# shizukutanaka/Otedama

Measured on AMD Instinct MI355X. Metric: hashes/sec (whole node) SHA-256d + scrypt at 1/2/4/8 MI355X; p50 share latency, higher is better.
Workload: dtype u32

## Files before the change

### csrc/bindings.cpp

```cpp
#include <pybind11/pybind11.h>
#include <pybind11/stl.h>

#include <array>
#include <atomic>
#include <cstring>
#include <stdexcept>
#include <thread>
#include <tuple>

#include "otedama/aead.h"
#include "otedama/job.h"
#include "otedama/runtime.h"
#include "otedama/trace.h"
#include "otedama/sha256.h"
#include "otedama/sv2_frame.h"
#include "otedama/clock_bounds.h"
#include "otedama/launch_plan.h"
#include "otedama/search_launch.h"
#include "otedama/share_job.h"
#include "otedama/work_queue.h"
#include "otedama/x11.h"

namespace py = pybind11;
using namespace otedama;

namespace {

std::string need(const py::bytes& b, size_t n, const char* what) {
  std::string s = b;
  if (s.size() != n) throw std::invalid_argument(std::string(what) + ": expected " + std::to_string(n) + " bytes");
  return s;
}

py::bytes to_bytes(const uint8_t* p, size_t n) { return py::bytes(reinterpret_cast<const char*>(p), n); }

std::shared_ptr<JobTemplate> make_job(const py::dict& d) {
  auto j = std::make_shared<JobTemplate>();
  auto get = [&](const char* k) -> py::object {
    if (d.contains(k)) return py::object(d[k]);
    return py::none();
  };
  std::string hdr = need(d["header"].cast<py::bytes>(), 80, "header");
  std::memcpy(j->header, hdr.data(), 80);
  std::string tgt = need(d["target"].cast<py::bytes>(), 32, "target");
  std::memcpy(j->target, tgt.data(), 32);
  if (!get("epoch").is_none()) j->epoch = d["epoch"].cast<uint64_t>();
  if (!get("job_id").is_none()) j->job_id = d["job_id"].cast<std::string>();
  if (!get("channel_id").is_none()) j->channel_id = d["channel_id"].cast<uint32_t>();
  if (!get("algo").is_none()) {
    auto a = d["algo"].cast<std::string>();
    if (a == "sha256d") j->algo = Algo::kSha256d;
    else if (a == "scrypt") j->algo = Algo::kScrypt;
    else if (a == "x11") j->algo = Algo::kX11;
    else throw std::invalid_argument("unsupported algo for the native miner: " + a);
  }
  if (!get("version_mask").is_none()) j->version_mask = d["version_mask"].cast<uint32_t>();
  if (!get("ntime_roll").is_none()) j->ntime_roll = d["ntime_roll"].cast<uint32_t>();
  if (!get("coinb1").is_none()) {
    j->has_coinbase = true;
    std::string c1 = d["coinb1"].cast<py::bytes>(), c2 = d["coinb2"].cast<py::bytes>();
    std::string e1 = d["extranonce1"].cast<py::bytes>();
    j->coinb1.assign(c1.begin(), c1.end());
    j->coinb2.assign(c2.begin(), c2.end());
    j->extranonce1.assign(e1.begin(), e1.end());
    j->extranonce2_size = d["extranonce2_size"].cast<uint32_t>();
    for (auto& br : d["merkle_branches"].cast<py::list>()) {
      std::string b = br.cast<py::bytes>();
      j->merkle_branches.emplace_back(b.begin(), b.end());
    }
  }
  if (!get("variant_start").is_none()) j->variant_start = d["variant_start"].cast<uint64_t>();
  if (!get("variant_stride").is_none()) j->variant_stride = d["variant_stride"].cast<uint64_t>();
  if (j->variant_stride == 0) j->variant_stride = 1;
  return j;
}

py::list shares_to_list(std::vector<ShareRecord>&& v) {
  py::list out;
  for (auto& s : v) {
    py::dict d;
    d["epoch"] = s.epoch;
    d["job_id"] = s.job_id;
    d["channel_id"] = s.channel_id;
    d["nonce"] = s.nonce;
    d["ntime"] = s.ntime;
    d["version"] = s.version;
    d["extranonce2"] = s.extranonce2;
    d["extranonce2_size"] = s.extranonce2_size;
    d["hash"] = to_bytes(s.hash, 32);
    d["device_id"] = s.device_id;
    d["found_at"] = s.found_at;
    d["device_found_at"] = s.device_found_at;
    out.append(d);
  }
  return out;
}

py::dict stats_to_dict(const MinerStats& s) {
  py::dict d;
  d["hashes"] = s.hashes;
  d["candidates"] = s.candidates;
  d["shares"] = s.shares;
  d["dropped"] = s.dropped;
  d["launches"] = s.launches;
  d["rejected_candidates"] = s.rejected_candidates;
  d["variant_launches"] = s.variant_launches;
  d["busy_seconds"] = s.busy_seconds;
  d["faulted"] = s.faulted;
  d["error"] = s.error;
  d["variant_next"] = s.variant_next;
  d["variant_epoch"] = s.variant_epoch;
  d["job_switches"] = s.job_switches;
  d["last_job_switch_ms"] = s.last_job_switch_ms;
  d["job_switch_ms"] = s.job_switch_ms;
  d["work_started"] = s.work_started;
  d["reserved_cus"] = s.reserved_cus;
  d["ring_overflow"] = s.ring_overflow;
  d["verify_dropped"] = s.verify_dropped;
  d["verify_queue_peak"] = s.verify_queue_peak;
  d["launch_hashes"] = s.launch_hashes;
  d["aborted_launches"] = s.aborted_launches;
  d["ring_hits"] = s.ring_hits;
  d["clock_calib_rtt_us"] = s.clock_calib_rtt_us;
  d["clock_samples"] = s.clock_samples;
  d["host_abort"] = s.host_abort;
  d["hashes_done_at_s"] = s.hashes_done_at_s;
  {
    py::dict ph;
    for (const auto& kv : s.startup_ms) ph[py::str(kv.first)] = kv.second;
    d["startup_ms"] = ph;
    py::dict rs;
    for (const auto& kv : s.startup_rss_mb) rs[py::str(kv.first)] = kv.second;
    d["startup_rss_mb"] = rs;
  }
  return d;
}

}

PYBIND11_MODULE(_native, m) {
  m.doc() = "Otedama MI355X native runtime (gfx950 HIP kernels + C++ host runtime)";

  m.def("cpu_has_sha_ni", &cpu_has_sha_ni);
  m.def("sha256", [](const py::bytes& b) {
    std::string s = b; uint8_t o[32];
    sha256(reinterpret_cast<const uint8_t*>(s.data()), s.size(), o);
    return to_bytes(o, 32);
  });
  m.def("sha256d", [](const py::bytes& b) {
    std::string s = b; uint8_t o[32];
    { py::gil_scoped_release r; sha256d(reinterpret_cast<const uint8_t*>(s.data()), s.size(), o); }
    return to_bytes(o, 32);
  });
  m.def("hmac_sha256", [](const py::bytes& k, const py::bytes& msg) {
    std::string ks = k, ms = msg; uint8_t o[32];
    hmac_sha256(reinterpret_cast<const uint8_t*>(ks.data()), ks.size(),
                reinterpret_cast<const uint8_t*>(ms.data()), ms.size(), o);
    return to_bytes(o, 32);
  });
  m.def("aead_seal", [](int kind, const py::bytes& key, const py::bytes& nonce, const py::bytes& plain,
                        const py::bytes& aad) {
    std::string out = aead_seal(static_cast<AeadKind>(kind), key, nonce, plain, aad);
    return py::bytes(out);
  }, py::arg("kind"), py::arg("key"), py::arg("nonce"), py::arg("plain"), py::arg("aad") = py::bytes());
  m.def("aead_open", [](int kind, const py::bytes& key, const py::bytes& nonce, const py::bytes& sealed,
                        const py::bytes& aad) -> py::object {
    std::string out;
    if (!aead_open(static_cast<AeadKind>(kind), key, nonce, sealed, aad, &out)) return py::none();
    return py::bytes(out);
  }, py::arg("kind"), py::arg("key"), py::arg("nonce"), py::arg("sealed"), py::arg("aad") = py::bytes());
  m.attr("SCRYPT_COOP") = kScryptCoop;
  m.attr("SCRYPT_LANE_W8") = kScryptLaneW8;
  m.attr("SCRYPT_COOP2") = kScryptCoop2;
  m.attr("SCRYPT_COOP_SPLIT") = kScryptCoopSplit;
  m.attr("AEAD_AES256GCM") = 0;
  m.attr("AEAD_CHACHA20POLY1305") = 1;
  m.def("scrypt_1024_1_1_batch", [](const std::vector<py::bytes>& hs) {
    std::vector<std::string> in;
    for (const auto& h : hs) in.push_back(need(h, 80, "header"));
    std::vector<std::array<uint8_t, 32>> out(in.size());
    std::vector<const uint8_t*> ip;
    std::vector<uint8_t*> op;
    for (size_t i = 0; i < in.size(); ++i) {
      ip.push_back(reinterpret_cast<const uint8_t*>(in[i].data()));
      op.push_back(out[i].data());
    }
    {
      py::gil_scoped_release r;
      scrypt_1024_1_1_batch(int(in.size()), ip.data(), op.data());
    }
    py::list res;
    for (const auto& o : out) res.append(to_bytes(o.data(), 32));
    return res;
  });
  m.def("scrypt_1024_1_1", [](const py::bytes& h) {
    std::string s = need(h, 80, "header"); uint8_t o[32];
    { py::gil_scoped_release r; scrypt_1024_1_1(reinterpret_cast<const uint8_t*>(s.data()), o); }
    return to_bytes(o, 32);
  });
  m.def("_clock_bounds", [](double window, const std::vector<std::pair<double, double>>& samples) {
    ClockBounds cb(window);
    std::vector<double> out;
    for (const auto& s : samples) out.push_back(cb.add(s.first, s.second));
    return out;
  });
  m.def("_launch_plan_rules", [](uint64_t batch_nonces, uint32_t target_hi, bool capped, int sha_variants, int run,
                                 const std::string& reserve_cus, int ncu) {
    const ShaLayout lay = pick_layout(sha_variants, run);
    const CuMask cm = parse_reserved_cus(reserve_cus.c_str(), ncu);
    py::dict d;
    d["batch"] = normalize_batch(batch_nonces);
    d["cap"] = launch_cap_hashes(target_hi, capped);
    d["layout"] = py::make_tuple(lay.nvar, lay.use_v);
    d["cu_mask"] = cm.words;
    d["reserved"] = cm.reserved;
    return d;
  }, py::arg("batch_nonces") = 0, py::arg("target_hi") = 0, py::arg("capped") = true, py::arg("sha_variants") = 1,
     py::arg("run") = 1, py::arg("reserve_cus") = "", py::arg("ncu") = 256);
  m.def("_launch_plan_walk", [](const std::string& kind, uint64_t batch, uint64_t cap, int nvar, uint64_t lanes,
                                uint64_t start, size_t max_launches, uint64_t variant_start, uint64_t variant_stride) {
    const LaunchKind lk = kind == "scrypt" ? LaunchKind::kScrypt : kind == "x11" ? LaunchKind::kX11
                        : kind == "v" ? LaunchKind::kVersionParallel : kind == "k" ? LaunchKind::kVariantK
                        : kind == "single" ? LaunchKind::kSingle
                        : throw std::invalid_argument("kind: scrypt, x11, v, k or single");
    if (start >= kNonceSpace) throw std::invalid_argument("start must be below 2^32");
    SearchCursor c;
    c.nonce_off = start;
    std::vector<std::tuple<uint64_t, uint64_t, uint64_t>> launches;
    while (c.k == 0 && launches.size() < max_launches) {
      const uint64_t base = c.nonce_off, count = launch_count(lk, batch, cap, nvar, lanes, c.nonce_off);
      c.advance(count, nvar);
      launches.emplace_back(base, count, c.variant_next(variant_start, variant_stride, nvar));
    }
    return py::make_tuple(launches, c.k);
  }, py::arg("kind"), py::arg("batch"), py::arg("cap"), py::arg("nvar") = 1, py::arg("lanes") = 0,
     py::arg("start") = 0, py::arg("max_launches") = size_t(1) << 20, py::arg("variant_start") = 0,
     py::arg("variant_stride") = 1);
  m.def("_work_queue_flood", [](size_t cap, size_t n, bool hash_each, size_t batch) {
    BoundedWorkQueue<std::array<uint8_t, 80>> q(cap);
    std::atomic<uint64_t> processed{0};
    uint64_t accepted = 0;
    {
      py::gil_scoped_release r;
      std::thread consumer([&] {
        if (batch > 1) {
          std::vector<std::array<uint8_t, 80>> items;
          std::vector<const uint8_t*> ip;
          std::vector<std::array<uint8_t, 32>> outs(batch);
          std::vector<uint8_t*> op;
          for (auto& o : outs) op.push_back(o.data());
          while (items.clear(), q.pop_many(&items, batch) > 0) {
            ip.clear();
            for (const auto& it : items) ip.push_back(it.data());
            if (hash_each) scrypt_1024_1_1_batch(int(items.size()), ip.data(), op.data());
            processed.fetch_add(items.size());
          }
          return;
        }
        std::array<uint8_t, 80> h;
        uint8_t out[32];
        while (q.pop(&h)) {
          if (hash_each) scrypt_1024_1_1(h.data(), out);
          processed.fetch_add(1);
        }
      });
      for (size_t i = 0; i < n; ++i) {
        std::array<uint8_t, 80> h{};
        std::memcpy(h.data() + 76, &i, 4);
        if (q.push(std::move(h))) ++accepted;
      }
      q.stop(~size_t(0));
      consumer.join();
    }
    py::dict d;
    d["accepted"] = accepted;
    d["refused"] = q.refused();
    d["peak"] = q.peak();
    d["processed"] = processed.load();
    return d;
  }, py::arg("cap"), py::arg("n"), py::arg("hash_each") = true, py::arg("batch") = 1);
  m.attr("X11_STAGES") = kX11StageCount;
  m.def("x11", [](const py::bytes& msg) {
    std::string s = msg; uint8_t o[32];
    { py::gil_scoped_release r; x11::x11(reinterpret_cast<const uint8_t*>(s.data()), s.size(), o, nullptr); }
    return to_bytes(o, 32);
  }, py::arg("msg"));
  m.def("x11_trace", [](const py::bytes& msg) {
    std::string s = msg; uint8_t o[32], t[64 * kX11StageCount];
    x11::x11(reinterpret_cast<const uint8_t*>(s.data()), s.size(), o, t);
    return to_bytes(t, sizeof t);
  }, py::arg("msg"), "The 11 intermediate 64-byte digests of the X11 chain, concatenated.");
  m.def("x11_stage", [](int i, const py::bytes& msg) {
    if (i < 0 || i >= kX11StageCount) throw std::invalid_argument("stage must be in [0, 11)");
    std::string s = msg; uint8_t o[64];
    x11::stage(i, reinterpret_cast<const uint8_t*>(s.data()), s.size(), o);
    return to_bytes(o, 64);
  }, py::arg("stage"), py::arg("msg"));
  m.def("x11_luffa_sbox_selfcheck", &x11::luffa_sbox_selfcheck);
  m.def(
      "sv2_scan",
      [](py::buffer b, uint32_t max_frame) {
        py::buffer_info info = b.request();
        if (info.itemsize != 1 || info.ndim != 1) throw std::invalid_argument("sv2_scan: need a contiguous byte buffer");
        const size_t n = (size_t)info.size;
        if (n > 0xFFFFFFFFull) throw std::invalid_argument("sv2_scan: buffer larger than 4 GiB");
        std::vector<Sv2FrameRec> recs(n / kSv2HeaderSize + 1);
        size_t consumed = 0, k = 0;
        int status = kSv2Ok;
        {
          py::gil_scoped_release nogil;
          k = sv2_scan(static_cast<const uint8_t*>(info.ptr), n, max_frame, recs.data(), recs.size(), &consumed,
                       &status);
        }
        py::list frames(k);
        for (size_t i = 0; i < k; ++i) {
          const Sv2FrameRec& r = recs[i];
          frames[i] = py::make_tuple(r.extension_type, r.msg_type, r.offset, r.length);
        }
        return py::make_tuple(frames, consumed, status);
      },
      py::arg("buf"), py::arg("max_frame"),
      "Split complete SV2 frames: ([(extension_type, msg_type, payload_offset, payload_length)], consumed, status)");
  m.def("cpu_scan_sha256d", [](const py::bytes& h, const py::bytes& t, uint32_t start, uint64_t count) {
    std::string hs = need(h, 80, "header"), ts = need(t, 32, "target");
    std::vector<uint32_t> hits;
    {
      py::gil_scoped_release r;
      hits = cpu_scan_sha256d(reinterpret_cast<const uint8_t*>(hs.data()), reinterpret_cast<const uint8_t*>(ts.data()),
                              start, count);
    }
    return hits;
  }, py::arg("header"), py::arg("target"), py::arg("start"), py::arg("count"));
  m.def("cpu_scan_method", &cpu_scan_method);
  m.def("_cpu_scan_lanes", [](int lanes, const py::bytes& h, const py::bytes& t, uint32_t start, uint64_t count) {
    std::string hs = need(h, 80, "header"), ts = need(t, 32, "target");
    std::vector<uint32_t> hits;
    {
      py::gil_scoped_release r;
      hits = cpu_scan_sha256d_lanes(lanes, reinterpret_cast<const uint8_t*>(hs.data()),
                                    reinterpret_cast<const uint8_t*>(ts.data()), start, count);
    }
    return hits;
  });
  m.def("merkle_root", [](const py::dict& job, uint64_t en2) {
    auto j = make_job(job); uint8_t root[32];
    merkle_root_from_coinbase(*j, en2, root);
    return to_bytes(root, 32);
  });
  m.def("variant_header", [](const py::dict& job, uint64_t v) {
    auto j = make_job(job);
    uint8_t hdr[80]; uint32_t ver, nt; uint64_t en2;
    j->variant_header(v, hdr, &ver, &nt, &en2);
// ... 218 lines not shown
```

### csrc/kernels/cdna_bitops.h

```cpp
#pragma once
#include <hip/hip_runtime.h>

#include <cstdint>

namespace otedama_dev {

__device__ __forceinline__ uint32_t ror(uint32_t x, uint32_t n) { return __builtin_amdgcn_alignbit(x, x, n); }
__device__ __forceinline__ uint32_t rol(uint32_t x, uint32_t n) { return __builtin_amdgcn_alignbit(x, x, 32 - n); }

__device__ __forceinline__ uint32_t xor3(uint32_t a, uint32_t b, uint32_t c, bool lane_varying = true) {
  if (lane_varying) {
    uint32_t r;
    asm("v_bitop3_b32 %0, %1, %2, %3 bitop3:0x96" : "=v"(r) : "v"(a), "v"(b), "v"(c));
    return r;
  }
  return a ^ b ^ c;
}
__device__ __forceinline__ uint32_t ch(uint32_t e, uint32_t f, uint32_t g) {
  uint32_t r;
  asm("v_bitop3_b32 %0, %1, %2, %3 bitop3:0xca" : "=v"(r) : "v"(e), "v"(f), "v"(g));
  return r;
}
__device__ __forceinline__ uint32_t maj(uint32_t a, uint32_t b, uint32_t c) {
  uint32_t r;
  asm("v_bitop3_b32 %0, %1, %2, %3 bitop3:0xe8" : "=v"(r) : "v"(a), "v"(b), "v"(c));
  return r;
}

__device__ __forceinline__ uint32_t bS0(uint32_t a) { return xor3(ror(a, 2), ror(a, 13), ror(a, 22)); }
__device__ __forceinline__ uint32_t bS1(uint32_t e) { return xor3(ror(e, 6), ror(e, 11), ror(e, 25)); }
__device__ __forceinline__ uint32_t ss0(uint32_t x, bool v = true) { return xor3(ror(x, 7), ror(x, 18), x >> 3, v); }
__device__ __forceinline__ uint32_t ss1(uint32_t x, bool v = true) { return xor3(ror(x, 17), ror(x, 19), x >> 10, v); }

__device__ __forceinline__ constexpr uint32_t sha256_k(int i) {
  constexpr uint32_t k[64] = {
      0x428a2f98, 0x71374491, 0xb5c0fbcf, 0xe9b5dba5, 0x3956c25b, 0x59f111f1, 0x923f82a4, 0xab1c5ed5,
      0xd807aa98, 0x12835b01, 0x243185be, 0x550c7dc3, 0x72be5d74, 0x80deb1fe, 0x9bdc06a7, 0xc19bf174,
      0xe49b69c1, 0xefbe4786, 0x0fc19dc6, 0x240ca1cc, 0x2de92c6f, 0x4a7484aa, 0x5cb0a9dc, 0x76f988da,
      0x983e5152, 0xa831c66d, 0xb00327c8, 0xbf597fc7, 0xc6e00bf3, 0xd5a79147, 0x06ca6351, 0x14292967,
      0x27b70a85, 0x2e1b2138, 0x4d2c6dfc, 0x53380d13, 0x650a7354, 0x766a0abb, 0x81c2c92e, 0x92722c85,
      0xa2bfe8a1, 0xa81a664b, 0xc24b8b70, 0xc76c51a3, 0xd192e819, 0xd6990624, 0xf40e3585, 0x106aa070,
      0x19a4c116, 0x1e376c08, 0x2748774c, 0x34b0bcb5, 0x391c0cb3, 0x4ed8aa4a, 0x5b9cca4f, 0x682e6ff3,
      0x748f82ee, 0x78a5636f, 0x84c87814, 0x8cc70208, 0x90befffa, 0xa4506ceb, 0xbef9a3f7, 0xc67178f2};
  return k[i];
}

constexpr uint32_t kSha256IVd[8] = {0x6a09e667, 0xbb67ae85, 0x3c6ef372, 0xa54ff53a,
                                    0x510e527f, 0x9b05688c, 0x1f83d9ab, 0x5be0cd19};

__device__ __forceinline__ void sha256_compress(uint32_t st[8], const uint32_t msg[16]) {
  uint32_t W[64];
#pragma unroll
  for (int i = 0; i < 16; ++i) W[i] = msg[i];
  uint32_t a = st[0], b = st[1], c = st[2], d = st[3], e = st[4], f = st[5], g = st[6], h = st[7];
#pragma unroll
  for (int t = 0; t < 64; ++t) {
    if (t >= 16) W[t] = ss1(W[t - 2]) + W[t - 7] + ss0(W[t - 15]) + W[t - 16];
    const uint32_t t1 = h + bS1(e) + ch(e, f, g) + (sha256_k(t) + W[t]);
    const uint32_t t2 = bS0(a) + maj(a, b, c);
    h = g; g = f; f = e; e = d + t1; d = c; c = b; b = a; a = t1 + t2;
  }
  st[0] += a; st[1] += b; st[2] += c; st[3] += d; st[4] += e; st[5] += f; st[6] += g; st[7] += h;
}

}
```

### csrc/kernels/scrypt_search.hip

```cpp
#include <hip/hip_runtime.h>

#include <cstdint>

#include "cdna_bitops.h"
#include "hitsink_dev.h"
#include "scrypt_pbkdf_dev.h"
#include <cstdlib>
#include <cstring>

#include "otedama/job.h"
#include "otedama/search_launch.h"

namespace {

using namespace otedama_dev;
using namespace otedama_dev::scryptk;

__device__ __forceinline__ void salsa20_8(uint32_t B[16]) {
  uint32_t x0 = B[0], x1 = B[1], x2 = B[2], x3 = B[3], x4 = B[4], x5 = B[5], x6 = B[6], x7 = B[7];
  uint32_t x8 = B[8], x9 = B[9], x10 = B[10], x11 = B[11], x12 = B[12], x13 = B[13], x14 = B[14], x15 = B[15];
#pragma unroll
  for (int i = 0; i < 8; i += 2) {
    x4 ^= rol(x0 + x12, 7);   x8 ^= rol(x4 + x0, 9);    x12 ^= rol(x8 + x4, 13);   x0 ^= rol(x12 + x8, 18);
    x9 ^= rol(x5 + x1, 7);    x13 ^= rol(x9 + x5, 9);   x1 ^= rol(x13 + x9, 13);   x5 ^= rol(x1 + x13, 18);
    x14 ^= rol(x10 + x6, 7);  x2 ^= rol(x14 + x10, 9);  x6 ^= rol(x2 + x14, 13);   x10 ^= rol(x6 + x2, 18);
    x3 ^= rol(x15 + x11, 7);  x7 ^= rol(x3 + x15, 9);   x11 ^= rol(x7 + x3, 13);   x15 ^= rol(x11 + x7, 18);
    x1 ^= rol(x0 + x3, 7);    x2 ^= rol(x1 + x0, 9);    x3 ^= rol(x2 + x1, 13);    x0 ^= rol(x3 + x2, 18);
    x6 ^= rol(x5 + x4, 7);    x7 ^= rol(x6 + x5, 9);    x4 ^= rol(x7 + x6, 13);    x5 ^= rol(x4 + x7, 18);
    x11 ^= rol(x10 + x9, 7);  x8 ^= rol(x11 + x10, 9);  x9 ^= rol(x8 + x11, 13);   x10 ^= rol(x9 + x8, 18);
    x12 ^= rol(x15 + x14, 7); x13 ^= rol(x12 + x15, 9); x14 ^= rol(x13 + x12, 13); x15 ^= rol(x14 + x13, 18);
  }
  B[0] += x0; B[1] += x1; B[2] += x2; B[3] += x3; B[4] += x4; B[5] += x5; B[6] += x6; B[7] += x7;
  B[8] += x8; B[9] += x9; B[10] += x10; B[11] += x11; B[12] += x12; B[13] += x13; B[14] += x14; B[15] += x15;
}

__device__ __forceinline__ void blockmix(uint32_t X[32]) {
#pragma unroll
  for (int k = 0; k < 16; ++k) X[k] ^= X[16 + k];
  salsa20_8(X);
#pragma unroll
  for (int k = 0; k < 16; ++k) X[16 + k] ^= X[k];
  salsa20_8(X + 16);
}

template <int GAP>
__device__ __forceinline__ void scrypt_romix(uint32_t X[32], uint4* __restrict__ Vw, uint32_t lane) {
  for (int i = 0; i < 1024; ++i) {
    if (i % GAP == 0) store_entry(Vw + ((uint64_t(i / GAP) * 64u + lane) << 3), X);
    blockmix(X);
  }
  for (int i = 0; i < 1024; ++i) {
    const uint32_t j = X[16] & 1023u;
    uint32_t T[32];
    load_entry(Vw + ((uint64_t(j / GAP) * 64u + lane) << 3), T);
    if constexpr (GAP > 1) {
      for (uint32_t r = 0; r < (j % GAP); ++r) blockmix(T);
    }
#pragma unroll
    for (int k = 0; k < 32; ++k) X[k] ^= T[k];
    blockmix(X);
  }
}

typedef __attribute__((address_space(3))) void glds_lptr_t;
typedef unsigned coop_v4u __attribute__((ext_vector_type(4)));

#ifndef OTD_SCRYPT_STORE_CPOL
#define OTD_SCRYPT_STORE_CPOL 2
#endif
constexpr int kStoreNT = OTD_SCRYPT_STORE_CPOL;

__device__ __forceinline__ uint32_t coop_swz(uint32_t s_local) {
  return ((s_local >> 1) & 3u) | (((s_local >> 3) & 1u) << 2);
}

__device__ __forceinline__ void coop_store_entry(const uint32_t X[32], __amdgpu_buffer_rsrc_t rs, uint4* __restrict__ tile,
                                                 uint32_t lane, uint32_t i) {
  char* tb = reinterpret_cast<char*>(tile);
  uint32_t ln = lane;
  asm volatile("" : "+v"(ln));
  const uint32_t slot = ln & 7u, octet = ln >> 3, own = ln & 31u;
  const uint32_t rd = (own << 7) ^ (coop_swz(own) << 4);
#pragma unroll
  for (int h = 0; h < 2; ++h) {
    asm volatile("s_waitcnt lgkmcnt(0)" ::: "memory");
    if ((ln >> 5) == uint32_t(h)) {
#pragma unroll
      for (int c = 0; c < 8; ++c)
        *reinterpret_cast<uint4*>(tb + (rd ^ (uint32_t(c) << 4))) =
            make_uint4(X[4 * c], X[4 * c + 1], X[4 * c + 2], X[4 * c + 3]);
    }
    __builtin_amdgcn_wave_barrier();
#pragma unroll
    for (int r = 0; r < 4; ++r) {
      const uint4 v = tile[64 * r + ln];
      const uint32_t owner = uint32_t(32 * h + 8 * r) + octet;
      const uint32_t chunk = slot ^ (((octet >> 1) & 3u) | (uint32_t(r & 1) << 2));
      const coop_v4u vv = {v.x, v.y, v.z, v.w};
      __builtin_amdgcn_raw_buffer_store_b128(vv, rs, (i << 13) | (owner << 7) | (chunk << 4), 0, kStoreNT);
    }
  }
}

template <int LCPOL>
__device__ __forceinline__ void coop_issue(const uint32_t X[32], __amdgpu_buffer_rsrc_t rs, uint4* __restrict__ tile,
                                           uint32_t lane, coop_v4u R[4]) {
  uint32_t ln = lane;
  asm volatile("" : "+v"(ln));
  const uint32_t slot = ln & 7u, octet = ln >> 3;
  const uint32_t j = X[16] & 1023u;
  asm volatile("s_waitcnt lgkmcnt(0)" ::: "memory");
#pragma unroll
  for (int r = 0; r < 4; ++r) {
    const uint32_t chunk = slot ^ (((octet >> 1) & 3u) | (uint32_t(r & 1) << 2));
    const uint32_t o0 = uint32_t(8 * r) + octet, o1 = o0 + 32u;
    const uint32_t j0 = uint32_t(__shfl(int(j), int(o0), 64));
    const uint32_t j1 = uint32_t(__shfl(int(j), int(o1), 64));
    __builtin_amdgcn_raw_ptr_buffer_load_lds(rs, (glds_lptr_t*)(tile + 64 * r), 16, (j0 << 13) | (o0 << 7) | (chunk << 4),
                                             0, 0, LCPOL);
    R[r] = __builtin_amdgcn_raw_buffer_load_b128(rs, (j1 << 13) | (o1 << 7) | (chunk << 4), 0, LCPOL);
  }
}

__device__ __forceinline__ void coop_consume(uint32_t X[32], uint4* __restrict__ tile, uint32_t lane,
                                             const coop_v4u R[4]) {
  const char* tb = reinterpret_cast<const char*>(tile);
  uint32_t ln = lane;
  asm volatile("" : "+v"(ln));
  const uint32_t own = ln & 31u;
  const uint32_t rd = (own << 7) ^ (coop_swz(own) << 4);
  asm volatile("s_waitcnt vmcnt(0)" ::: "memory");
  if (ln < 32u) {
#pragma unroll
    for (int c = 0; c < 8; ++c) {
      const uint4 t = *reinterpret_cast<const uint4*>(tb + (rd ^ (uint32_t(c) << 4)));
      X[4 * c] ^= t.x; X[4 * c + 1] ^= t.y; X[4 * c + 2] ^= t.z; X[4 * c + 3] ^= t.w;
    }
  }
  asm volatile("s_waitcnt lgkmcnt(0)" ::: "memory");
#pragma unroll
  for (int r = 0; r < 4; ++r) tile[64 * r + ln] = make_uint4(R[r].x, R[r].y, R[r].z, R[r].w);
  __builtin_amdgcn_wave_barrier();
  if (ln >= 32u) {
#pragma unroll
    for (int c = 0; c < 8; ++c) {
      const uint4 t = *reinterpret_cast<const uint4*>(tb + (rd ^ (uint32_t(c) << 4)));
      X[4 * c] ^= t.x; X[4 * c + 1] ^= t.y; X[4 * c + 2] ^= t.z; X[4 * c + 3] ^= t.w;
    }
  }
}

template <int LCPOL, int POLL>
__device__ __forceinline__ bool scrypt_romix_coop(uint32_t X[32], __amdgpu_buffer_rsrc_t rs, uint4* __restrict__ tile,
                                                  uint32_t lane, const otedama::HitSink& sink) {
  static_assert(POLL > 0 && 1024 % POLL == 0, "poll interval must divide the ROMix loop");
  if (abort_newer(abort_peek(sink), sink.epoch)) return false;
  for (uint32_t c = 0; c < 1024; c += POLL) {
    if (c && abort_newer(abort_peek_scalar(sink), sink.epoch)) return false;
    for (uint32_t i = c; i < c + POLL; ++i) {
      coop_store_entry(X, rs, tile, lane, i);
      blockmix(X);
    }
  }
  if (abort_newer(abort_peek(sink), sink.epoch)) return false;
  for (int i = 0; i < 1024; ++i) {
    coop_v4u R[4];
    coop_issue<LCPOL>(X, rs, tile, lane, R);
    coop_consume(X, tile, lane, R);
    blockmix(X);
  }
  return true;
}

template <int LCPOL, int PHASE>
__device__ __forceinline__ void scrypt_romix_coop_phase(uint32_t X[32], __amdgpu_buffer_rsrc_t rs,
                                                        uint4* __restrict__ tile, uint32_t lane) {
  if constexpr (PHASE == 1) {
    for (uint32_t i = 0; i < 1024; ++i) {
      coop_store_entry(X, rs, tile, lane, i);
      blockmix(X);
    }
  } else {
    for (int i = 0; i < 1024; ++i) {
      coop_v4u R[4];
      coop_issue<LCPOL>(X, rs, tile, lane, R);
      coop_consume(X, tile, lane, R);
      blockmix(X);
    }
  }
}

template <int LCPOL>
__device__ __forceinline__ void scrypt_romix_coop2(uint32_t XA[32], uint32_t XB[32], __amdgpu_buffer_rsrc_t rsA,
                                                   __amdgpu_buffer_rsrc_t rsB, uint4* __restrict__ tile, uint32_t lane) {
  for (uint32_t i = 0; i < 1024; ++i) {
    coop_store_entry(XA, rsA, tile, lane, i);
    blockmix(XA);
    coop_store_entry(XB, rsB, tile, lane, i);
    blockmix(XB);
  }
  coop_v4u R[4];
  coop_issue<LCPOL>(XA, rsA, tile, lane, R);
  for (int i = 0; i < 1024; ++i) {
    coop_consume(XA, tile, lane, R);
    coop_issue<LCPOL>(XB, rsB, tile, lane, R);
    blockmix(XA);
    coop_consume(XB, tile, lane, R);
    if (i < 1023) coop_issue<LCPOL>(XA, rsA, tile, lane, R);
    blockmix(XB);
  }
}

}

extern "C" __global__ __launch_bounds__(256) void otd_scrypt_pbkdf_in(const otedama::ScryptParams p, uint32_t base,
                                                                      uint32_t count, uint4* __restrict__ xbuf) {
  const uint32_t i = blockIdx.x * blockDim.x + threadIdx.x;
  if (i >= count) return;
  uint32_t X[32];
  scrypt_pbkdf_in(p, base + i, X);
  store_entry(xbuf + (uint64_t(i) << 3), X);
}

template <int GAP>
__global__ __launch_bounds__(256) void otd_scrypt_romix(uint32_t count, uint4* __restrict__ xbuf,
                                                        uint4* __restrict__ V) {
  const uint64_t slot = uint64_t(blockIdx.x) * blockDim.x + threadIdx.x;
  const uint64_t nslots = uint64_t(gridDim.x) * blockDim.x;
  uint4* Vw = V + (slot >> 6) * (uint64_t(1024 / GAP) * 64u * 8u);
  const uint32_t lane = uint32_t(slot & 63u);
  for (uint64_t i = slot; i < count; i += nslots) {
    uint32_t X[32];
    load_entry(xbuf + (i << 3), X);
    scrypt_romix<GAP>(X, Vw, lane);
    store_entry(xbuf + (i << 3), X);
  }
}

template <int LCPOL, int POLL>
__global__ __launch_bounds__(256) __attribute__((amdgpu_waves_per_eu(8, 8))) void otd_scrypt_romix_coop(uint32_t count, uint4* __restrict__ xbuf,
                                                             uint4* __restrict__ V, const otedama::HitSink sink) {
  __shared__ uint4 tiles[4 * 256];
  const uint64_t slot = uint64_t(blockIdx.x) * blockDim.x + threadIdx.x;
  const uint64_t nslots = uint64_t(gridDim.x) * blockDim.x;
  const uint32_t lane = uint32_t(slot & 63u);
  const uint64_t wave = (uint64_t(__builtin_amdgcn_readfirstlane(uint32_t(slot >> 32))) << 26) |
                        uint64_t(__builtin_amdgcn_readfirstlane(uint32_t(slot) >> 6));
  uint4* Vw = V + wave * (1024ull * 64u * 8u);
  const __amdgpu_buffer_rsrc_t rs = __builtin_amdgcn_make_buffer_rsrc(Vw, (short)0, 1024 * 64 * 128, 0x00020000);
  (void)Vw;
  uint4* tile = tiles + __builtin_amdgcn_readfirstlane(threadIdx.x >> 6) * 256;
  for (uint64_t i = slot; i < count; i += nslots) {
    uint32_t X[32];
    load_entry(xbuf + (i << 3), X);
    if (!scrypt_romix_coop<LCPOL, POLL>(X, rs, tile, lane, sink)) return;
    store_entry(xbuf + (i << 3), X);
  }
}

template <int LCPOL, int PHASE>
__global__ __launch_bounds__(256) __attribute__((amdgpu_waves_per_eu(8, 8))) void otd_scrypt_romix_coop_phase(
    uint32_t count, uint4* __restrict__ xbuf, uint4* __restrict__ V) {
  __shared__ uint4 tiles[4 * 256];
  const uint64_t slot = uint64_t(blockIdx.x) * blockDim.x + threadIdx.x;
  const uint32_t lane = uint32_t(slot & 63u);
  const uint64_t wave = (uint64_t(__builtin_amdgcn_readfirstlane(uint32_t(slot >> 32))) << 26) |
                        uint64_t(__builtin_amdgcn_readfirstlane(uint32_t(slot) >> 6));
  uint4* Vw = V + wave * (1024ull * 64u * 8u);
  const __amdgpu_buffer_rsrc_t rs = __builtin_amdgcn_make_buffer_rsrc(Vw, (short)0, 1024 * 64 * 128, 0x00020000);
  uint4* tile = tiles + __builtin_amdgcn_readfirstlane(threadIdx.x >> 6) * 256;
  if (slot < count) {
    uint32_t X[32];
    load_entry(xbuf + (slot << 3), X);
    scrypt_romix_coop_phase<LCPOL, PHASE>(X, rs, tile, lane);
    store_entry(xbuf + (slot << 3), X);
  }
}

template <int LCPOL>
__global__ __launch_bounds__(256) __attribute__((amdgpu_waves_per_eu(8, 8))) void otd_scrypt_romix_coop_seg(
    uint32_t count, uint4* __restrict__ xbuf, uint4* __restrict__ V, uint32_t it0, uint32_t it1,
    const otedama::HitSink sink) {
  __shared__ uint4 tiles[4 * 256];
  const uint64_t slot = uint64_t(blockIdx.x) * blockDim.x + threadIdx.x;
  const uint32_t lane = uint32_t(slot & 63u);
  uint4* tile = tiles + __builtin_amdgcn_readfirstlane(threadIdx.x >> 6) * 256;
  if (abort_newer(abort_peek(sink), sink.epoch)) return;
  const uint64_t nslots = uint64_t(gridDim.x) * blockDim.x;
  for (uint64_t h = slot; h < count; h += nslots) {
    const uint64_t hw = (uint64_t(__builtin_amdgcn_readfirstlane(uint32_t(h >> 32))) << 26) |
                        uint64_t(__builtin_amdgcn_readfirstlane(uint32_t(h) >> 6));
    const __amdgpu_buffer_rsrc_t rh =
        __builtin_amdgcn_make_buffer_rsrc(V + hw * (1024ull * 64u * 8u), (short)0, 1024 * 64 * 128, 0x00020000);
    uint32_t X[32];
    load_entry(xbuf + (h << 3), X);
    const uint32_t w1 = it1 < 1024u ? it1 : 1024u;
    for (uint32_t i = it0; i < w1; ++i) {
      coop_store_entry(X, rh, tile, lane, i);
      blockmix(X);
    }
    for (uint32_t i = it0 > 1024u ? it0 : 1024u; i < it1; ++i) {
      coop_v4u R[4];
      coop_issue<LCPOL>(X, rh, tile, lane, R);
      coop_consume(X, tile, lane, R);
      blockmix(X);
    }
    store_entry(xbuf + (h << 3), X);
  }
}

template <int LCPOL>
__global__ __launch_bounds__(256) __attribute__((amdgpu_waves_per_eu(4, 4))) void otd_scrypt_romix_coop2(
    uint32_t count, uint4* __restrict__ xbuf, uint4* __restrict__ V) {
  __shared__ uint4 tiles[4 * 256];
  const uint32_t lane = threadIdx.x & 63u;
  const uint64_t wave0 = (uint64_t(blockIdx.x) * blockDim.x + threadIdx.x) >> 6;
  const uint64_t nwaves = (uint64_t(gridDim.x) * blockDim.x) >> 6;
  const uint64_t wslot = (uint64_t(__builtin_amdgcn_readfirstlane(uint32_t(wave0 >> 32))) << 32) |
                         uint64_t(__builtin_amdgcn_readfirstlane(uint32_t(wave0)));
  uint4* VA = V + wslot * (2ull * 1024 * 64 * 8);
  uint4* VB = VA + 1024ull * 64 * 8;
  const __amdgpu_buffer_rsrc_t rsA = __builtin_amdgcn_make_buffer_rsrc(VA, (short)0, 1024 * 64 * 128, 0x00020000);
  const __amdgpu_buffer_rsrc_t rsB = __builtin_amdgcn_make_buffer_rsrc(VB, (short)0, 1024 * 64 * 128, 0x00020000);
  uint4* tile = tiles + __builtin_amdgcn_readfirstlane(threadIdx.x >> 6) * 256;
  for (uint64_t w = wslot; w * 128 < count; w += nwaves) {
    const uint64_t ia = w * 128 + lane, ib = ia + 64;
    uint32_t XA[32], XB[32];
    load_entry(xbuf + (ia << 3), XA);
    load_entry(xbuf + (ib << 3), XB);
    scrypt_romix_coop2<LCPOL>(XA, XB, rsA, rsB, tile, lane);
    store_entry(xbuf + (ia << 3), XA);
    store_entry(xbuf + (ib << 3), XB);
  }
}

__global__ __launch_bounds__(256) __attribute__((amdgpu_waves_per_eu(8, 8))) void otd_scrypt_romix_w8(
    uint32_t count, uint4* __restrict__ xbuf, uint4* __restrict__ V) {
  const uint64_t slot = uint64_t(blockIdx.x) * blockDim.x + threadIdx.x;
  const uint64_t nslots = uint64_t(gridDim.x) * blockDim.x;
  uint4* Vw = V + (slot >> 6) * (1024ull * 64u * 8u);
  const uint32_t lane = uint32_t(slot & 63u);
  for (uint64_t i = slot; i < count; i += nslots) {
    uint32_t X[32];
    load_entry(xbuf + (i << 3), X);
    scrypt_romix<1>(X, Vw, lane);
    store_entry(xbuf + (i << 3), X);
  }
}

extern "C" __global__ __launch_bounds__(256) void otd_scrypt_pbkdf_out(const otedama::ScryptParams p, uint32_t base,
                                                                       uint32_t count, const uint4* __restrict__ xbuf,
                                                                       const otedama::HitSink sink) {
  const uint32_t i = blockIdx.x * blockDim.x + threadIdx.x;
  if (i >= count) return;
  if (abort_newer(abort_peek(sink), sink.epoch)) return;
  uint32_t X[32];
  load_entry(xbuf + (uint64_t(i) << 3), X);
  const uint32_t h7 = scrypt_pbkdf_out(p, base + i, X);
  if (bswap(h7) <= p.target_hi) hit_publish(sink, base + i, 0u);
}

template __global__ void otd_scrypt_romix<1>(uint32_t, uint4*, uint4*);
template __global__ void otd_scrypt_romix<2>(uint32_t, uint4*, uint4*);
template __global__ void otd_scrypt_romix<4>(uint32_t, uint4*, uint4*);

namespace otedama {

uint64_t scrypt_scratch_bytes(int grid, int gap) {
  if (gap == kScryptCoop2) return uint64_t(grid) * 512ull * 1024ull * 128ull;
  if (gap == kScryptCoop || gap == kScryptLaneW8 || gap == kScryptCoopSplit) gap = 1;
  return uint64_t(grid) * 256ull * (1024ull / uint64_t(gap)) * 128ull;
}

static bool scrypt_write_polls() {
  static const bool on = [] {
    const char* v = std::getenv("OTEDAMA_SCRYPT_POLL");
    return !(v && v[0] == '0');
  }();
  return on;
}

static uint32_t scrypt_segments() {
  const char* v = std::getenv("OTEDAMA_SCRYPT_SEGMENTS");
  if (!v || !v[0]) return 0;
  const long x = std::strtol(v, nullptr, 10);
  return uint32_t(x < 1 ? 1 : (x > 64 ? 64 : x));
}

static int scrypt_seg_grid(int grid) {
  const char* v = std::getenv("OTEDAMA_SCRYPT_SEG_GRID");
  if (!v || !v[0]) return grid;
  int cap = 0;
  if (std::strcmp(v, "resident") == 0) {
    int dev = 0, cus = 0;
    if (hipGetDevice(&dev) != hipSuccess ||
        hipDeviceGetAttribute(&cus, hipDeviceAttributeMultiprocessorCount, dev) != hipSuccess || cus <= 0)
      return grid;
    cap = cus * 8;
  } else {
    cap = int(std::strtol(v, nullptr, 10));
  }
  return cap > 0 && cap < grid ? cap : grid;
}

hipError_t launch_scrypt_romix(uint32_t count, uint4* X, uint4* V, int gap, const HitSink& sink, int grid,
                               hipStream_t stream) {
  const uint32_t count64 = (count + 63u) & ~63u;
  switch (gap) {
    case kScryptCoop:
      if (scrypt_segments() > 0 && uint64_t(count64) <= uint64_t(grid) * 256u) {
        const uint32_t S = scrypt_segments();
        const int sg = scrypt_seg_grid(grid);
        for (uint32_t k = 0; k < S; ++k)
          hipLaunchKernelGGL(otd_scrypt_romix_coop_seg<2>, dim3(sg), dim3(256), 0, stream, count64, X, V,
                             2048u * k / S, 2048u * (k + 1) / S, sink);
      } else if (scrypt_write_polls())
        hipLaunchKernelGGL((otd_scrypt_romix_coop<2, 64>), dim3(grid), dim3(256), 0, stream, count64, X, V, sink);
      else
        hipLaunchKernelGGL((otd_scrypt_romix_coop<2, 1024>), dim3(grid), dim3(256), 0, stream, count64, X, V, sink);
      break;
    case kScryptLaneW8:
      hipLaunchKernelGGL(otd_scrypt_romix_w8, dim3(grid), dim3(256), 0, stream, count, X, V);
      break;
    case kScryptCoopSplit:
      hipLaunchKernelGGL((otd_scrypt_romix_coop_phase<2, 1>), dim3(grid), dim3(256), 0, stream, count64, X, V);
      hipLaunchKernelGGL((otd_scrypt_romix_coop_phase<2, 2>), dim3(grid), dim3(256), 0, stream, count64, X, V);
      break;
    case kScryptCoop2:
      hipLaunchKernelGGL(otd_scrypt_romix_coop2<2>, dim3(grid), dim3(256), 0, stream, (count + 127u) & ~127u, X, V);
      break;
    case 1: hipLaunchKernelGGL(otd_scrypt_romix<1>, dim3(grid), dim3(256), 0, stream, count, X, V); break;
    case 2: hipLaunchKernelGGL(otd_scrypt_romix<2>, dim3(grid), dim3(256), 0, stream, count, X, V); break;
    case 4: hipLaunchKernelGGL(otd_scrypt_romix<4>, dim3(grid), dim3(256), 0, stream, count, X, V); break;
    default: return hipErrorInvalidValue;
  }
  return hipSuccess;
}

hipError_t launch_scrypt_search(const ScryptParams& p, uint32_t base, uint32_t count, void* xbuf, void* scratch,
                                int gap, const HitSink& sink, int grid, hipStream_t stream) {
  uint4* X = static_cast<uint4*>(xbuf);
  uint4* V = static_cast<uint4*>(scratch);
  const int eg = int((count + 255) / 256);
  if (gap == kScryptCoopSplit && uint64_t((count + 63u) & ~63u) > uint64_t(grid) * 256u) return hipErrorInvalidValue;
  hipLaunchKernelGGL(otd_scrypt_pbkdf_in, dim3(eg), dim3(256), 0, stream, p, base, count, X);
  if (launch_scrypt_romix(count, X, V, gap, sink, grid, stream) != hipSuccess) return hipErrorInvalidValue;
  hipLaunchKernelGGL(otd_scrypt_pbkdf_out, dim3(eg), dim3(256), 0, stream, p, base, count, X, sink);
  return hipGetLastError();
}

}
```

Measured before the change: 19.46 billion.

## Schedule Salsa20/8 with deferred XORs and fuse ROMix entry XOR into blockmix

Salsa20/8 becomes a compile-time scheduled form. Some XOR updates are held pending and later folded into v_xad_u32 (xor-then-add) or three-input XOR instructions, cutting the VALU op count per quarter-round. The ROMix second-loop XOR of the fetched V entry is fused with blockmix's initial X[k]^=X[16+k] through xor3 in coop_consume, so the mixed blockmix variant skips that pass. A static_assert checks the legality of the pending schedule, and a host binding exposes both forms for testing. The cost is more live registers for the pending values, which may affect occupancy.

```diff
diff --git a/csrc/bindings.cpp b/csrc/bindings.cpp
--- a/csrc/bindings.cpp
+++ b/csrc/bindings.cpp
@@ -11,6 +11,7 @@
 #include "otedama/aead.h"
 #include "otedama/job.h"
 #include "otedama/runtime.h"
+#include "otedama/salsa_sched.h"
 #include "otedama/trace.h"
 #include "otedama/sha256.h"
 #include "otedama/sv2_frame.h"
@@ -198,6 +199,16 @@
     { py::gil_scoped_release r; scrypt_1024_1_1(reinterpret_cast<const uint8_t*>(s.data()), o); }
     return to_bytes(o, 32);
   });
+  m.def("_salsa20_8", [](const py::bytes& block, const std::string& form) {
+    std::string s = need(block, 64, "block");
+    uint32_t B[16];
+    std::memcpy(B, s.data(), 64);
+    if (form == "sched") otedama_salsa::salsa20_8_sched<otedama_salsa::PlainOps>(B);
+    else if (form == "plain") otedama_salsa::salsa20_8_plain<otedama_salsa::PlainOps>(B);
+    else throw std::invalid_argument("form: sched or plain");
+    return to_bytes(reinterpret_cast<const uint8_t*>(B), 64);
+  }, py::arg("block"), py::arg("form"));
+  m.attr("_SALSA_PENDING_XORS") = otedama_salsa::pending_count();
   m.def("_clock_bounds", [](double window, const std::vector<std::pair<double, double>>& samples) {
     ClockBounds cb(window);
     std::vector<double> out;
diff --git a/csrc/include/otedama/salsa_sched.h b/csrc/include/otedama/salsa_sched.h
--- /dev/null
+++ b/csrc/include/otedama/salsa_sched.h
@@ -0,0 +1,115 @@
+#pragma once
+#include <cstdint>
+
+#if defined(__HIPCC__)
+#define OTD_SALSA_FN __host__ __device__ __forceinline__
+#else
+#define OTD_SALSA_FN inline
+#endif
+
+namespace otedama_salsa {
+
+struct Update {
+  uint8_t t, a, b, rot;
+};
+
+OTD_SALSA_FN constexpr Update salsa_update(int i) {
+  constexpr Update k[32] = {
+      {4, 0, 12, 7},   {8, 4, 0, 9},    {12, 8, 4, 13},   {0, 12, 8, 18},   {9, 5, 1, 7},    {13, 9, 5, 9},
+      {1, 13, 9, 13},  {5, 1, 13, 18},  {14, 10, 6, 7},   {2, 14, 10, 9},   {6, 2, 14, 13},  {10, 6, 2, 18},
+      {3, 15, 11, 7},  {7, 3, 15, 9},   {11, 7, 3, 13},   {15, 11, 7, 18},  {1, 0, 3, 7},    {2, 1, 0, 9},
+      {3, 2, 1, 13},   {0, 3, 2, 18},   {6, 5, 4, 7},     {7, 6, 5, 9},     {4, 7, 6, 13},   {5, 4, 7, 18},
+      {11, 10, 9, 7},  {8, 11, 10, 9},  {9, 8, 11, 13},   {10, 9, 8, 18},   {12, 15, 14, 7}, {13, 12, 15, 9},
+      {14, 13, 12, 13}, {15, 14, 13, 18}};
+  return k[i];
+}
+
+#ifndef OTD_SALSA_PENDING
+#define OTD_SALSA_PENDING 0x9a6a, 0x4515, 0xb0e0, 0x4e1b, 0xa1a4, 0x4e1b, 0x2184, 0xde7b
+#endif
+OTD_SALSA_FN constexpr uint32_t pending_mask(int r) {
+  constexpr uint16_t m[8] = {OTD_SALSA_PENDING};
+  return m[r];
+}
+
+constexpr bool pending_set_legal() {
+  uint32_t pend = 0;
+  for (int u = 0; u < 128; ++u) {
+    const Update x = salsa_update(u % 32);
+    if ((pend >> x.a) & (pend >> x.b) & 1u) return false;
+    if ((pending_mask(u / 16) >> x.t) & 1u) {
+      if ((pend >> x.t) & 1u) return false;
+      pend |= 1u << x.t;
+    } else {
+      pend &= ~(1u << x.t);
+    }
+  }
+  return true;
+}
+static_assert(pending_set_legal(), "OTD_SALSA_PENDING breaks a rule of the pending-xor schedule");
+
+constexpr int pending_count() {
+  int n = 0;
+  for (int r = 0; r < 8; ++r)
+    for (int w = 0; w < 16; ++w) n += (pending_mask(r) >> w) & 1;
+  return n;
+}
+
+struct PlainOps {
+  static OTD_SALSA_FN uint32_t rol(uint32_t x, uint32_t n) { return (x << n) | (x >> (32u - n)); }
+  static OTD_SALSA_FN uint32_t xad(uint32_t a, uint32_t b, uint32_t c) { return (a ^ b) + c; }
+  static OTD_SALSA_FN uint32_t xor3(uint32_t a, uint32_t b, uint32_t c) { return a ^ b ^ c; }
+};
+
+template <class Ops>
+OTD_SALSA_FN void salsa20_8_plain(uint32_t B[16]) {
+  uint32_t x[16];
+#pragma unroll
+  for (int i = 0; i < 16; ++i) x[i] = B[i];
+#pragma unroll
+  for (int u = 0; u < 128; ++u) {
+    const Update k = salsa_update(u % 32);
+    x[k.t] ^= Ops::rol(x[k.a] + x[k.b], k.rot);
+  }
+#pragma unroll
+  for (int i = 0; i < 16; ++i) B[i] += x[i];
+}
+
+template <class Ops>
+OTD_SALSA_FN void salsa20_8_sched(uint32_t B[16]) {
+  uint32_t v[16], p[16];
+#pragma unroll
+  for (int i = 0; i < 16; ++i) {
+    v[i] = B[i];
+    p[i] = 0;
+  }
+  uint32_t pend = 0;
+#pragma unroll
+  for (int r = 0; r < 8; ++r) {
+#pragma unroll
+    for (int q = 0; q < 16; ++q) {
+      const Update k = salsa_update((r & 1) * 16 + q);
+      uint32_t s;
+      if ((pend >> k.a) & 1u)
+        s = Ops::xad(v[k.a], p[k.a], v[k.b]);
+      else if ((pend >> k.b) & 1u)
+        s = Ops::xad(v[k.b], p[k.b], v[k.a]);
+      else
+        s = v[k.a] + v[k.b];
+      const uint32_t rt = Ops::rol(s, k.rot);
+      if ((pend >> k.t) & 1u) {
+        v[k.t] = Ops::xor3(v[k.t], p[k.t], rt);
+        pend &= ~(1u << k.t);
+      } else if ((pending_mask(r) >> k.t) & 1u) {
+        p[k.t] = rt;
+        pend |= 1u << k.t;
+      } else {
+        v[k.t] ^= rt;
+      }
+    }
+  }
+#pragma unroll
+  for (int i = 0; i < 16; ++i) B[i] = ((pend >> i) & 1u) ? Ops::xad(v[i], p[i], B[i]) : B[i] + v[i];
+}
+
+}
diff --git a/csrc/kernels/cdna_bitops.h b/csrc/kernels/cdna_bitops.h
--- a/csrc/kernels/cdna_bitops.h
+++ b/csrc/kernels/cdna_bitops.h
@@ -15,6 +15,11 @@
     return r;
   }
   return a ^ b ^ c;
+}
+__device__ __forceinline__ uint32_t xad(uint32_t a, uint32_t b, uint32_t c) {
+  uint32_t r;
+  asm("v_xad_u32 %0, %1, %2, %3" : "=v"(r) : "v"(a), "v"(b), "v"(c));
+  return r;
 }
 __device__ __forceinline__ uint32_t ch(uint32_t e, uint32_t f, uint32_t g) {
   uint32_t r;
diff --git a/csrc/kernels/scrypt_search.hip b/csrc/kernels/scrypt_search.hip
--- a/csrc/kernels/scrypt_search.hip
+++ b/csrc/kernels/scrypt_search.hip
@@ -9,6 +9,7 @@
 #include <cstring>
 
 #include "otedama/job.h"
+#include "otedama/salsa_sched.h"
 #include "otedama/search_launch.h"
 
 namespace {
@@ -16,31 +17,36 @@
 using namespace otedama_dev;
 using namespace otedama_dev::scryptk;
 
-__device__ __forceinline__ void salsa20_8(uint32_t B[16]) {
-  uint32_t x0 = B[0], x1 = B[1], x2 = B[2], x3 = B[3], x4 = B[4], x5 = B[5], x6 = B[6], x7 = B[7];
-  uint32_t x8 = B[8], x9 = B[9], x10 = B[10], x11 = B[11], x12 = B[12], x13 = B[13], x14 = B[14], x15 = B[15];
-#pragma unroll
-  for (int i = 0; i < 8; i += 2) {
-    x4 ^= rol(x0 + x12, 7);   x8 ^= rol(x4 + x0, 9);    x12 ^= rol(x8 + x4, 13);   x0 ^= rol(x12 + x8, 18);
-    x9 ^= rol(x5 + x1, 7);    x13 ^= rol(x9 + x5, 9);   x1 ^= rol(x13 + x9, 13);   x5 ^= rol(x1 + x13, 18);
-    x14 ^= rol(x10 + x6, 7);  x2 ^= rol(x14 + x10, 9);  x6 ^= rol(x2 + x14, 13);   x10 ^= rol(x6 + x2, 18);
-    x3 ^= rol(x15 + x11, 7);  x7 ^= rol(x3 + x15, 9);   x11 ^= rol(x7 + x3, 13);   x15 ^= rol(x11 + x7, 18);
-    x1 ^= rol(x0 + x3, 7);    x2 ^= rol(x1 + x0, 9);    x3 ^= rol(x2 + x1, 13);    x0 ^= rol(x3 + x2, 18);
-    x6 ^= rol(x5 + x4, 7);    x7 ^= rol(x6 + x5, 9);    x4 ^= rol(x7 + x6, 13);    x5 ^= rol(x4 + x7, 18);
-    x11 ^= rol(x10 + x9, 7);  x8 ^= rol(x11 + x10, 9);  x9 ^= rol(x8 + x11, 13);   x10 ^= rol(x9 + x8, 18);
-    x12 ^= rol(x15 + x14, 7); x13 ^= rol(x12 + x15, 9); x14 ^= rol(x13 + x12, 13); x15 ^= rol(x14 + x13, 18);
-  }
-  B[0] += x0; B[1] += x1; B[2] += x2; B[3] += x3; B[4] += x4; B[5] += x5; B[6] += x6; B[7] += x7;
-  B[8] += x8; B[9] += x9; B[10] += x10; B[11] += x11; B[12] += x12; B[13] += x13; B[14] += x14; B[15] += x15;
-}
-
-__device__ __forceinline__ void blockmix(uint32_t X[32]) {
-#pragma unroll
-  for (int k = 0; k < 16; ++k) X[k] ^= X[16 + k];
+struct SalsaDevOps {
+  static __device__ __forceinline__ uint32_t rol(uint32_t x, uint32_t n) { return otedama_dev::rol(x, n); }
+  static __device__ __forceinline__ uint32_t xad(uint32_t a, uint32_t b, uint32_t c) { return otedama_dev::xad(a, b, c); }
+  static __device__ __forceinline__ uint32_t xor3(uint32_t a, uint32_t b, uint32_t c) { return otedama_dev::xor3(a, b, c); }
+};
+
+__device__ __forceinline__ void salsa20_8(uint32_t B[16]) { otedama_salsa::salsa20_8_sched<SalsaDevOps>(B); }
+
+__device__ __forceinline__ void blockmix_mixed(uint32_t X[32]) {
   salsa20_8(X);
 #pragma unroll
   for (int k = 0; k < 16; ++k) X[16 + k] ^= X[k];
   salsa20_8(X + 16);
+}
+
+__device__ __forceinline__ void blockmix(uint32_t X[32]) {
+#pragma unroll
+  for (int k = 0; k < 16; ++k) X[k] ^= X[16 + k];
+  blockmix_mixed(X);
+}
+
+__device__ __forceinline__ void xor_entry_mix(uint32_t X[32], int c, uint4 t) {
+  if (c >= 4) {
+    X[4 * c] ^= t.x; X[4 * c + 1] ^= t.y; X[4 * c + 2] ^= t.z; X[4 * c + 3] ^= t.w;
+  } else {
+    X[4 * c] = xor3(X[4 * c], t.x, X[4 * c + 16]);
+    X[4 * c + 1] = xor3(X[4 * c + 1], t.y, X[4 * c + 17]);
+    X[4 * c + 2] = xor3(X[4 * c + 2], t.z, X[4 * c + 18]);
+    X[4 * c + 3] = xor3(X[4 * c + 3], t.w, X[4 * c + 19]);
+  }
 }
 
 template <int GAP>
@@ -132,10 +138,8 @@
   asm volatile("s_waitcnt vmcnt(0)" ::: "memory");
   if (ln < 32u) {
 #pragma unroll
-    for (int c = 0; c < 8; ++c) {
-      const uint4 t = *reinterpret_cast<const uint4*>(tb + (rd ^ (uint32_t(c) << 4)));
-      X[4 * c] ^= t.x; X[4 * c + 1] ^= t.y; X[4 * c + 2] ^= t.z; X[4 * c + 3] ^= t.w;
-    }
+    for (int c = 7; c >= 0; --c)
+      xor_entry_mix(X, c, *reinterpret_cast<const uint4*>(tb + (rd ^ (uint32_t(c) << 4))));
   }
   asm volatile("s_waitcnt lgkmcnt(0)" ::: "memory");
 #pragma unroll
@@ -143,10 +147,8 @@
   __builtin_amdgcn_wave_barrier();
   if (ln >= 32u) {
 #pragma unroll
-    for (int c = 0; c < 8; ++c) {
-      const uint4 t = *reinterpret_cast<const uint4*>(tb + (rd ^ (uint32_t(c) << 4)));
-      X[4 * c] ^= t.x; X[4 * c + 1] ^= t.y; X[4 * c + 2] ^= t.z; X[4 * c + 3] ^= t.w;
-    }
+    for (int c = 7; c >= 0; --c)
+      xor_entry_mix(X, c, *reinterpret_cast<const uint4*>(tb + (rd ^ (uint32_t(c) << 4))));
   }
 }
 
@@ -167,7 +169,7 @@
     coop_v4u R[4];
     coop_issue<LCPOL>(X, rs, tile, lane, R);
     coop_consume(X, tile, lane, R);
-    blockmix(X);
+    blockmix_mixed(X);
   }
   return true;
 }
@@ -185,7 +187,7 @@
       coop_v4u R[4];
       coop_issue<LCPOL>(X, rs, tile, lane, R);
       coop_consume(X, tile, lane, R);
-      blockmix(X);
+      blockmix_mixed(X);
     }
   }
 }
@@ -204,10 +206,10 @@
   for (int i = 0; i < 1024; ++i) {
     coop_consume(XA, tile, lane, R);
     coop_issue<LCPOL>(XB, rsB, tile, lane, R);
-    blockmix(XA);
+    blockmix_mixed(XA);
     coop_consume(XB, tile, lane, R);
     if (i < 1023) coop_issue<LCPOL>(XA, rsA, tile, lane, R);
-    blockmix(XB);
+    blockmix_mixed(XB);
   }
 }
 
@@ -303,7 +305,7 @@
       coop_v4u R[4];
       coop_issue<LCPOL>(X, rh, tile, lane, R);
       coop_consume(X, tile, lane, R);
-      blockmix(X);
+      blockmix_mixed(X);
     }
     store_entry(xbuf + (h << 3), X);
   }
```

After: 19.44 billion. About the same (-0.1%).
